# robertknight/ocrs-models

Measured on AMD Instinct MI355X. Metric: detection train-step images/sec, higher is better.
Workload: dtype bf16

## Files before the change

### ocrs_models_amd/csrc/det_mm.hip

```cpp
#include "det_common.h"
#include "det_rs.h"
#include <type_traits>

constexpr int mf_th(int cin, int cout, int nst) { return (nst != 2 && cin == 8 && cout != 32) ? 16 : 8; }

namespace {

template <int C>
struct MmPitch {
    static constexpr int V = (C == 32) ? 40 : C;
};

template <int CIN, int COUT, bool PPOOL = false>
struct MmCfg {
    static constexpr bool N256 = CIN == 32 && (COUT == 32 || COUT == 16);
    static constexpr int NT = N256 ? 256 : 512, NW = NT / 64;
    static constexpr int BPC = 2;
    static constexpr int TW = 32;
    static constexpr int TH = (CIN == 32 || COUT == 32) ? 8 : ((CIN == 16 && COUT == 16 && !PPOOL) ? 8 : 12);
    static constexpr bool MERGE = N256;
    static constexpr int TP = TW * TH;
    static constexpr bool T12P = CIN == 16 && COUT == 16 && TH == 12;
    static constexpr bool BDB = !(CIN == 8 && COUT == 16 && TH == 12) && !T12P && !N256;
    static constexpr int DW_ = TW + 2, DH_ = TH + 2, DP = DW_ * DH_;
    static constexpr int CGI = CIN / 8, CGO = COUT / 8;
    static constexpr int PD = MmPitch<COUT>::V, PX = MmPitch<CIN>::V;
    static constexpr int MT = (CIN + 15) / 16, NTO = (COUT + 15) / 16;
    static constexpr int KC = (9 * COUT + 31) / 32;
    static constexpr int NPW = TP / 16 / NW;
    static constexpr int KS = TP / 32;
    static constexpr int TAPU = (COUT == 8) ? 5 : 9;
    static constexpr int NOWN = (TAPU == 9) ? 8 / NW : 1;
    static constexpr int NGI = (DP * CGO + NT - 1) / NT;
    static constexpr int NXI = (TP * CGI + NT - 1) / NT;
    static constexpr int NWIN = (DH_ / 2) * (DW_ / 2);
    static constexpr int NWI = (NWIN * 2 * CGO + NT - 1) / NT;
    static_assert(DH_ % 2 == 0 && NT % (2 * CGO) == 0 && 4 * NWI <= 16, "pooled item layout");
    static constexpr int OFF_D = 0;
    static constexpr int OFF_X = (OFF_D + DP * PD * 2 + 63) & ~63;
    static constexpr int OFF_WF = (OFF_X + TP * PX * 2 + 64 + 63) & ~63;
    static constexpr int OFF_PAR = OFF_WF + MT * KC * 64 * 16;
    static constexpr int PAR_FLOATS = 3 * CIN + 6 * COUT + 9 * CIN + COUT * CIN + NW * 2 * MT * 16;
    static constexpr int TILE_BYTES = OFF_PAR + PAR_FLOATS * 4;
    static constexpr int SLOT_FLOATS = (NW * NOWN * MT * NTO + NW) * 256 + NW * 2 * MT * 16;
    static constexpr int SMEM = TILE_BYTES > SLOT_FLOATS * 4 ? TILE_BYTES : SLOT_FLOATS * 4;
    static constexpr int PART = COUT * CIN + 9 * CIN + 2 * CIN;
};

__device__ __forceinline__ f32x4 mfma16(const uint4& a, const uint4& b, f32x4 c) {
    return __builtin_amdgcn_mfma_f32_16x16x32_bf16(__builtin_bit_cast(bf16x8, a), __builtin_bit_cast(bf16x8, b), c, 0, 0, 0);
}
__device__ __forceinline__ f32x4 mfma16(const bf16x8& a, const bf16x8& b, f32x4 c) { return __builtin_amdgcn_mfma_f32_16x16x32_bf16(a, b, c, 0, 0, 0); }

__device__ __forceinline__ void half4(const Raw8<bf16>& r, int hf, float (&v)[4]) {
    const unsigned a = hf ? r.a.z : r.a.x, b = hf ? r.a.w : r.a.y;
    v[0] = __uint_as_float(a << 16); v[1] = __uint_as_float(a & 0xffff0000u);
    v[2] = __uint_as_float(b << 16); v[3] = __uint_as_float(b & 0xffff0000u);
}
__device__ __forceinline__ void st4bf(bf16* p, const float (&v)[4]) {
    unsigned lo, hi;
    asm("v_cvt_pk_bf16_f32 %0, %1, %2" : "=v"(lo) : "v"(v[0]), "v"(v[1]));
    asm("v_cvt_pk_bf16_f32 %0, %1, %2" : "=v"(hi) : "v"(v[2]), "v"(v[3]));
    *reinterpret_cast<uint2*>(p) = make_uint2(lo, hi);
}

typedef unsigned u32x4 __attribute__((ext_vector_type(4)));
__device__ __forceinline__ u32x4 gload16_opaque(const void* p) {
    u32x4 r;
    asm volatile("global_load_dwordx4 %0, %1, off" : "=&v"(r) : "v"(p) : "memory");
    return r;
}
template <int N>
__device__ __forceinline__ void wait_vm_tied(u32x4& r) {
    static_assert(N >= 0 && N < 64, "vmcnt is a 6-bit field");
    asm volatile("s_waitcnt vmcnt(%1)" : "+v"(r) : "n"(N) : "memory");
}
template <int NL, int NS, int K = 0>
__device__ __forceinline__ void static_for_wait(u32x4* v) {
    if constexpr (K < NL) {
        wait_vm_tied<NS + NL - 1 - K>(v[K]);
        static_for_wait<NL, NS, K + 1>(v);
    }
}
__device__ __forceinline__ Raw8<bf16> raw8_of(const u32x4& v) {
    Raw8<bf16> r;
    r.a = make_uint4(v.x, v.y, v.z, v.w);
    return r;
}

template <int CINB, int COUT>
constexpr int mm_fwd_lb() { return (CINB == 16 && COUT == 8) ? 6 : 4; }
template <int CINB, int COUT>
constexpr bool mm_fwd_fink() { return !(CINB == 16 && COUT == 8); }
template <int CIN, int COUT, bool PPOOL>
constexpr int mm_bwd_lb() { return MmCfg<CIN, COUT, PPOOL>::BPC * MmCfg<CIN, COUT, PPOOL>::NW / 4; }
}

template <int CIN, int COUT, bool PPOOL, bool G2, bool STATS, bool FULL = false>
__global__ __launch_bounds__((MmCfg<CIN, COUT, PPOOL>::NT), (mm_bwd_lb<CIN, COUT, PPOOL>())) void k_mm_bwd(Src2<bf16> x, const float* __restrict__ tra, const float* __restrict__ trb,
                                                   const float* __restrict__ wdw ,
                                                   const float* __restrict__ wpw , int ldw,
                                                   const bf16* __restrict__ g1, const bf16* __restrict__ g2, const bf16* __restrict__ z,
                                                   const float* __restrict__ bn, const float* __restrict__ coef, bf16* __restrict__ gxa,
                                                   bf16* __restrict__ gxb, float* __restrict__ ws, Tiling2 tg, BnFin fin, BwdLast bl) {
    using C = MmCfg<CIN, COUT, PPOOL>;
    constexpr int NT = C::NT, TW = C::TW, TH = C::TH, TP = C::TP, DW_ = C::DW_, DP = C::DP, CGI = C::CGI, CGO = C::CGO, PD = C::PD, PX = C::PX;
    constexpr int MT = C::MT, NTO = C::NTO, KC = C::KC, NPW = C::NPW, KS = C::KS;
    static_assert(!(FULL && PPOOL), "pooled launches have border tiles by construction (origin shift)");
    extern __shared__ __attribute__((aligned(64))) char smem[];
    bf16* tileD = reinterpret_cast<bf16*>(smem + C::OFF_D);
    bf16* tileX = reinterpret_cast<bf16*>(smem + C::OFF_X);
    uint4* s_wf = reinterpret_cast<uint4*>(smem + C::OFF_WF);
    float* s_trx = reinterpret_cast<float*>(smem + C::OFF_PAR);
    float* s_bn = s_trx + 3 * CIN;
    float* s_cf = s_bn + 3 * COUT;
    float* s_w9 = s_cf + 3 * COUT;
    float* s_wp = s_w9 + 9 * CIN;
    const int H = tg.H, W = tg.W;
    const int tid = threadIdx.x, lane = tid & 63, l15 = lane & 15;
    const int wave = __builtin_amdgcn_readfirstlane(tid >> 6);

    fill_tr8(s_trx, x, tra, trb, CIN, tid);
    for (int i = tid; i < 3 * COUT; i += NT) s_bn[i] = bn[i];
    if (fin.gsum) {
        bn_fin_coef(fin, COUT, s_cf, tid, NT, blockIdx.x == 0);
    } else {
        for (int i = tid; i < 3 * COUT; i += NT) s_cf[i] = coef[i];
    }
    for (int i = tid; i < 9 * CIN; i += NT) s_w9[i] = wdw[i];
    for (int i = tid; i < COUT * CIN; i += NT) s_wp[i] = wpw[(i / CIN) * ldw + (i % CIN)];
    {
        const uint4 z4 = make_uint4(0, 0, 0, 0);
        for (int i = tid; i < C::OFF_WF / 16; i += NT) reinterpret_cast<uint4*>(smem)[i] = z4;
    }
    __syncthreads();
    for (int f = tid; f < MT * KC * 64; f += NT) {
        const int l = f & 63, kc = (f >> 6) % KC, mt = (f >> 6) / KC;
        const int m = (FULL && CIN == 8) ? (l & 7) : mt * 16 + (l & 15);
        float v[8];
#pragma unroll
        for (int j = 0; j < 8; ++j) {
            const int k = kc * 32 + (l >> 4) * 8 + j, tap = k / COUT, o = k % COUT;
            v[j] = (m < CIN && tap < 9) ? s_w9[m * 9 + tap] * s_wp[o * CIN + m] : 0.f;
        }
        s_wf[f] = make_uint4(pack2bf(v[0], v[1]), pack2bf(v[2], v[3]), pack2bf(v[4], v[5]), pack2bf(v[6], v[7]));
    }
    __syncthreads();

    const int cgo = tid % CGO;
    constexpr int NQ = 2 * CGO;
    const int cq4 = (tid % NQ) * 4;
    int gi_dyx[PPOOL ? C::NWI : C::NGI];
    if constexpr (!PPOOL) {
#pragma unroll
        for (int j = 0; j < C::NGI; ++j) {
            const int d = (tid + j * NT) / CGO, dy = d / DW_, dx = d - dy * DW_;
            gi_dyx[j] = dy | (dx << 16);
        }
    } else {
#pragma unroll
        for (int j = 0; j < C::NWI; ++j) {
            const int wd = (tid + j * NT) / NQ, wy = wd / (DW_ / 2), wx = wd - wy * (DW_ / 2);
            gi_dyx[j] = (2 * wy) | ((2 * wx) << 16);
        }
    }
    const int cgi = tid % CGI;
    const bool xi_a = cgi * 8 < x.Ca;
    const bf16* xi_base = xi_a ? x.a + cgi * 8 : x.b + (cgi * 8 - x.Ca);
    const int xi_pitch = xi_a ? x.Ca : x.Cb;
    constexpr int ORG = PPOOL ? -1 : 0;

    constexpr int NG = PPOOL ? 1 : C::NGI, NP = PPOOL ? C::NWI : 1;
    constexpr int GW = G2 ? 3 : 2, NLOADS = NG * GW + C::NXI;
    constexpr int PFD = 1;
    u32x4 pf[PFD][NLOADS];
    constexpr int NSTORE = NPW * MT;
    uint2 zp[4 * NP], gp1[NP], gp2[G2 ? NP : 1];
    unsigned okg_[PFD], okx_[PFD];
#pragma unroll
    for (int q = 0; q < PFD; ++q) okg_[q] = okx_[q] = 0;
    auto ld16 = [&](const bf16* p) -> u32x4 {
        if constexpr (FULL) {
            return gload16_opaque(p);
        } else {
            const uint4 q = *reinterpret_cast<const uint4*>(p);
            return (u32x4){q.x, q.y, q.z, q.w};
        }
    };
    auto issue = [&](const TileOrg& o, auto SET) {
        constexpr int SI = decltype(SET)::value;
        unsigned okg = 0, okx = 0;
        const int h00 = o.h0 + ORG - 1, w00 = o.w0 + ORG - 1;
        const int corner = (o.n * H + h00) * W + w00;
        const bf16* zb = z + (long)corner * COUT;
        const bool inside = FULL && h00 >= 0 && w00 >= 0 && h00 + C::DH_ <= H && w00 + DW_ <= W;
        if constexpr (!PPOOL) {
            const bf16* g1b = g1 + (long)corner * COUT;
            const bf16* g2b = (G2 ? g2 : g1) + (long)corner * COUT;
            auto items = [&](auto INSIDE) {
#pragma unroll
// ... 47 lines not shown
        else xitems(std::false_type{});
        okg_[SI] = okg;
        okx_[SI] = okx;
    };

    const int kg = lane >> 4;
    auto tap_off = [](int tap) constexpr -> int { return tap < 9 ? ((2 - tap / 3) * DW_ + (2 - tap % 3)) * PD : 0; };
    auto boff_of = [&](int kc, bool& valid) -> int {
        if constexpr (COUT == 32) {
            valid = true;
            return tap_off(kc) + kg * 8;
        } else if constexpr (COUT == 16) {
            const int t0 = 2 * kc, t1 = 2 * kc + 1;
            valid = (kg < 2) ? t0 < 9 : t1 < 9;
            return ((kg < 2) ? tap_off(t0) : tap_off(t1)) + (kg & 1) * 8;
        } else {
            const int t0 = 4 * kc;
            valid = t0 + kg < 9;
            const int a = (kg & 1) ? tap_off(t0 + 1) : tap_off(t0), b = (kg & 1) ? tap_off(t0 + 3) : tap_off(t0 + 2);
            return (kg & 2) ? b : a;
        }
    };
    const int prow = 4 * (lane >> 4) + ((lane & 15) >> 2), pcol = (lane & 3) * 4;
    auto unit_off = [&](int u) -> int {
        if constexpr (COUT == 8) {
            const int sel = (lane & 3) >> 1;
            int tap = 2 * u + sel;
            tap = tap > 8 ? 8 : tap;
            const int ky = tap / 3, kx = tap - ky * 3;
            return ((2 - ky) * DW_ + prow + 2 - kx) * PD + (lane & 1) * 4;
        } else {
            const int ky = u / 3, kx = u - ky * 3;
            return ((2 - ky) * DW_ + prow + 2 - kx) * PD + pcol;
        }
    };
    constexpr int NSUB = MT * NTO, NKR = C::NW / NSUB;
    static_assert(C::NW % NSUB == 0 && KS >= NKR, "shared-unit split");
    const int u_own = (C::TAPU == 9) ? wave : (wave & 3);
    const int ks_own0 = (C::TAPU == 9) ? 0 : (wave >> 2) * (KS / 2), ks_own1 = (C::TAPU == 9) ? KS : ks_own0 + KS / 2;
    const int sh_a = (wave % NSUB) % MT, sh_b = (wave % NSUB) / MT, sh_k0 = (wave / NSUB) * KS / NKR, sh_k1 = (wave / NSUB + 1) * KS / NKR;
    constexpr int NOWN = C::NOWN;
    int off_own[NOWN];
#pragma unroll
    for (int j = 0; j < NOWN; ++j) off_own[j] = unit_off(u_own + j * C::NW);
    const int off_sh = unit_off(C::TAPU - 1) + sh_b * 16;
    f32x4 accO[NOWN][MT][NTO], accS = (f32x4){0.f, 0.f, 0.f, 0.f};
#pragma unroll
    for (int j = 0; j < NOWN; ++j)
#pragma unroll
        for (int a = 0; a < MT; ++a)
#pragma unroll
            for (int b = 0; b < NTO; ++b) accO[j][a][b] = (f32x4){0.f, 0.f, 0.f, 0.f};
    constexpr bool STL = STATS && (MT == 2 || C::T12P);
    float* s_st = s_wp + COUT * CIN;
    float st1[(STATS && !STL) ? MT : 1][4];
    if constexpr (STATS && !STL) {
#pragma unroll
        for (int a = 0; a < MT; ++a)
#pragma unroll
            for (int i = 0; i < 4; ++i) st1[a][i] = 0.f;
    }
    if constexpr (STL) {
        for (int i = tid; i < C::NW * 2 * MT * 16; i += NT) s_st[i] = 0.f;
    }

    TileSched ts(tg.ntiles);
    TileIter<TW, TH> tit(tg, ts.first < ts.end ? ts.first : 0, ts.step);
    TileOrg orgs[PFD];
    orgs[0] = tit.org();
    using I0 = std::integral_constant<int, 0>;
    if (ts.first < ts.end) issue(orgs[0], I0{});
    auto tile_body = [&](long t, auto KIND, auto SET) __attribute__((always_inline)) {
        constexpr int SI = decltype(SET)::value, KI = decltype(KIND)::value;
        const TileOrg org = orgs[SI];
        const unsigned okg = okg_[SI], okx = okx_[SI];
        if constexpr (FULL) {
            constexpr int YOUNGER = KI == 0 ? 0 : NSTORE;
            static_for_wait<NLOADS, YOUNGER>(pf[SI]);
        }
        if constexpr (!PPOOL) {
#pragma unroll
            for (int hf = 0; hf < 2; ++hf) {
                const int c4 = cgo * 8 + hf * 4;
                const f32x4 bs = *reinterpret_cast<const f32x4*>(s_bn + c4), bt = *reinterpret_cast<const f32x4*>(s_bn + COUT + c4);
                const f32x4 ca = *reinterpret_cast<const f32x4*>(s_cf + c4), cb = *reinterpret_cast<const f32x4*>(s_cf + COUT + c4),
                            cc = *reinterpret_cast<const f32x4*>(s_cf + 2 * COUT + c4);
#pragma unroll
                for (int j = 0; j < C::NGI; ++j) {
                    const int it = tid + j * NT;
                    if (DP * CGO % NT == 0 || it < DP * CGO) {
                        float dz[4] = {0.f, 0.f, 0.f, 0.f};
                        if (okg & (1u << j)) {
                            float zv[4], ga[4];
                            half4(raw8_of(pf[SI][j * GW + 0]), hf, zv);
                            half4(raw8_of(pf[SI][j * GW + 1]), hf, ga);
                            if constexpr (G2) {
                                float gb[4];
                                half4(raw8_of(pf[SI][j * GW + 2]), hf, gb);
#pragma unroll
                                for (int i = 0; i < 4; ++i) ga[i] += gb[i];
                            }
#pragma unroll
                            for (int i = 0; i < 4; ++i) {
                                const float gh = fmaf(zv[i], bs[i], bt[i]) > 0.f ? ga[i] : 0.f;
                                dz[i] = fmaf(ca[i], gh, fmaf(cb[i], zv[i], cc[i]));
                            }
                        }
// ... 340 lines not shown
    red[chain][col] = s;
    __syncthreads();
    __shared__ float fin[32];
    const float v = ((red[0][col] + red[1][col]) + (red[2][col] + red[3][col])) + ((red[4][col] + red[5][col]) + (red[6][col] + red[7][col]));
    if (chain == 0) fin[col] = v;
    __syncthreads();
    if (chain != 0 || e >= nelem) return;
    if (e >= COUT * CIN + 9 * CIN) {
        const int r2 = e - (COUT * CIN + 9 * CIN);
        if (r2 & 1) return;
        const int c = r2 >> 1, Cb = CIN - Ca;
        const bool in_a = c < Ca;
        double* gs = in_a ? gsum_a : gsum_b;
        if (!gs) return;
        const int cc = in_a ? c : c - Ca, Cs = in_a ? Ca : Cb;
        const float* sv = in_a ? saved_a : saved_b;
        const float* tr = in_a ? tra : trb;
        const double S1 = v, S2 = fin[col + 1], sc = tr[cc], sh = tr[Cs + cc], mean = sv[cc], rstd = sv[Cs + cc];
        gs[cc] += S1;
        if (sc != 0.0) gs[Cs + cc] += rstd * ((S2 - sh * S1) / sc - mean * S1);
        return;
    }
    if (e < COUT * CIN) {
        const int o = e / CIN, c = e - o * CIN;
        dwpw[o * ldw + c] += v;
        return;
    }
    const int r = e - COUT * CIN;
    if (r < 9 * CIN) {
        dwdw[r] += v;
        return;
    }
    return;
}
static int mm_grid(int th, int N, int H, int W, int pooled, int bpc = 2) {
    const long ntiles = (long)N * ((W + pooled + 31) / 32) * ((H + pooled + th - 1) / th);
    return persistent_grid(ntiles, bpc);
}
static int mm_bwd_th(int Cin, int Cout, int pooled) {
    if (Cin == 32 || Cout == 32) return 8;
    return (Cin == 16 && Cout == 16 && !pooled) ? 8 : 12;
}

template <int CIN, int COUT, bool PPOOL, bool G2, bool STATS>
static void mm_bwd_launch1(const Src2<bf16>& x, const float* tra, const float* trb, const float* wdw, const float* wpw, int ldw, const bf16* g1, const bf16* g2,
                           const bf16* z, const float* bn, const float* coef, bf16* gxa, bf16* gxb, float* ws, int N, int H, int W, int nb, const BnFin& fin,
                           const BwdLast& bl, hipStream_t st) {
    using CC = MmCfg<CIN, COUT, PPOOL>;
    Tiling2 tg = make_tiling2(N, H + (PPOOL ? 1 : 0), W + (PPOOL ? 1 : 0), CC::TW, CC::TH);
    tg.H = H;
    tg.W = W;
    if constexpr (!PPOOL) {
        if (W % CC::TW == 0) {
            hipFuncSetAttribute(reinterpret_cast<const void*>(&k_mm_bwd<CIN, COUT, PPOOL, G2, STATS, true>), hipFuncAttributeMaxDynamicSharedMemorySize, CC::SMEM);
            OCRS_LAUNCH_T((k_mm_bwd<CIN, COUT, PPOOL, G2, STATS, true>), dim3(nb), dim3(CC::NT), CC::SMEM, st, x, tra, trb, wdw, wpw, ldw, g1, g2, z, bn, coef,
                          gxa, gxb, ws, tg, fin, bl);
            return;
        }
    }
    hipFuncSetAttribute(reinterpret_cast<const void*>(&k_mm_bwd<CIN, COUT, PPOOL, G2, STATS, false>), hipFuncAttributeMaxDynamicSharedMemorySize, CC::SMEM);
    OCRS_LAUNCH_T((k_mm_bwd<CIN, COUT, PPOOL, G2, STATS, false>), dim3(nb), dim3(CC::NT), CC::SMEM, st, x, tra, trb, wdw, wpw, ldw, g1, g2, z, bn, coef, gxa, gxb,
                  ws, tg, fin, bl);
}

template <int CIN, int COUT>
static void mm_bwd_dispatch(const Src2<bf16>& x, const float* tra, const float* trb, const float* wdw, const float* wpw, int ldw, const bf16* g1, const bf16* g2,
                            int pooled, const bf16* z, const float* bn, const float* coef, bf16* gxa, bf16* gxb, float* ws, bool stats, int N, int H, int W,
                            int nb, const BnFin& fin, const BwdLast& bl, hipStream_t st) {
#define MMB(PP, GG, SS) mm_bwd_launch1<CIN, COUT, PP, GG, SS>(x, tra, trb, wdw, wpw, ldw, g1, g2, z, bn, coef, gxa, gxb, ws, N, H, W, nb, fin, bl, st)
    if (pooled) {
        if (g2) { if (stats) MMB(true, true, true); else MMB(true, true, false); }
        else    { if (stats) MMB(true, false, true); else MMB(true, false, false); }
    } else {
        if (g2) { if (stats) MMB(false, true, true); else MMB(false, true, false); }
        else    { if (stats) MMB(false, false, true); else MMB(false, false, false); }
    }
#undef MMB
}

static BwdLast mm_bwd_last(bool want, int Cin, int Ca, double* gsA, double* gsB, const float* svA, const float* svB) {
    BwdLast bl{nullptr, nullptr, gsA, gsB, svA, svB, Ca, 0};
    if (!want) return bl;
    double* p = bwd_defer_scratch(BWD_LAST_SLOTS * 2 * Cin + 2);
    if (p) {
        bl.raw = p;
        bl.counter = reinterpret_cast<unsigned*>(p + BWD_LAST_SLOTS * 2 * Cin);
    }
    return bl;
}
static void mm_bwd_second_stage(const float* ws, int nb, int Cin, int Cout, int Ca, float* dwpw, int ldw, float* dwdw, double* gsA, double* gsB, const float* svA,
                                const float* svB, const float* tA, const float* tB, const BwdLast& bl, bool may_defer, hipStream_t st) {
    const int ne = Cout * Cin + 11 * Cin;
    if (bl.raw) {
        gsA = gsB = nullptr;
        if (may_defer && bwd_defer_reduce(ws, nb, ne, dwpw, Cout * Cin, Cin, ldw, dwdw, 9 * Cin)) return;
    } else if (may_defer && !gsA && !gsB && bwd_defer_reduce(ws, nb, ne, dwpw, Cout * Cin, Cin, ldw, dwdw, 9 * Cin)) {
        return;
    }
    OCRS_LAUNCH_T(k_mm_bwd_reduce, dim3((ne + 31) / 32), dim3(256), 0, st, ws, nb, Cin, Cout, Ca, dwpw, ldw, dwdw, gsA, gsB, svA, svB, tA, tB);
}

extern "C" {

long ocrs_mm_bwd_supported(int Ca, int Cb, int Cout, int dtype) {
    if (dtype != 1 || !(Cout == 8 || Cout == 16 || Cout == 32)) return 0;
    const int Cin = Ca + Cb;
    if (Ca == 32 && Cb == 32) return 1;
    if ((Cin == 8 && Cout == 32) || (Cin == 32 && Cout == 8)) return 0;
    return (Cin == 8 || Cin == 16 || Cin == 32) && Ca % 8 == 0 && Cb % 8 == 0;
}
long ocrs_mm_bwd_ws_floats(int Ca, int Cb, int Cout, int N, int H, int W) {
    const int Cin = (Ca == 32 && Cb == 32) ? 32 : Ca + Cb;
    const int nb0 = mm_grid(mm_bwd_th(Cin, Cout, 0), N, H, W, 0), nb1 = mm_grid(mm_bwd_th(Cin, Cout, 1), N, H, W, 1);
    const long tiled = (long)(nb0 > nb1 ? nb0 : nb1) * (Cout * Cin + 11 * Cin + 1024) * ((Ca == 32 && Cb == 32) ? 2 : 1);
// ... 68 lines not shown
                       const float* bn, const double* gsum, const float* gamma, const float* saved, float* dgamma, float* dbeta, void* gxa, float* dwpw,
                       float* dwdw, float* ws, const float* saved_a, double* gsum_a, int Cout, int N, int H, int W, int dtype, hipStream_t st) {
    OCRS_CHECK_ARG(xu && wexp && tra && wdw && wpw && g1 && z && bn && gsum && gamma && saved && dgamma && dbeta && gxa && dwpw && dwdw && ws);
    OCRS_CHECK_ARG(ocrs_mm_bwd_head_supported(8, 0, Cout, N, H, W, dtype) && (!gsum_a || saved_a));
    const BnFin fin{gsum, gamma, saved, dgamma, dbeta, (long)N * H * W};
    Src2<bf16> x{nullptr, nullptr, 8, 0};
    const int nb = rs_bwd_blocks(8, Cout, N, H, W, g2 != nullptr);
    const BwdLast bl = mm_bwd_last(gsum_a != nullptr, 8, 8, gsum_a, nullptr, saved_a, nullptr);
    rs_bwd_launch(x, tra, nullptr, wdw, wpw, 8, (const bf16*)g1, (const bf16*)g2, (const bf16*)z, bn, nullptr, (bf16*)gxa, nullptr, ws, gsum_a != nullptr, Cout, N, H, W,
                  fin, st, nullptr, nullptr, (const bf16*)xu, wexp, bl);
    mm_bwd_second_stage(ws, nb, 8, Cout, 8, dwpw, 8, dwdw, gsum_a, nullptr, saved_a, nullptr, tra, nullptr, bl, true, st);
    OCRS_LAUNCH_CHECK();
    return OCRS_OK;
}

int ocrs_mm_bwd_fin_xu_c1(const void* xu, const float* wexp, const float* tra, const float* wdw, const float* wpw, const void* g1, const void* g2, const void* z,
                          const float* bn, const double* gsum, const float* gamma, const float* saved, float* dgamma, float* dbeta, float* dwpw, float* dwdw,
                          float* ws, const float* saved_a, double* gsum_a, const float* img, double* c1acc, int Cout, int N, int H, int W, int dtype,
                          hipStream_t st) {
    OCRS_CHECK_ARG(xu && wexp && tra && wdw && wpw && g1 && z && bn && gsum && gamma && saved && dgamma && dbeta && dwpw && dwdw && ws && img && c1acc);
    OCRS_CHECK_ARG(Cout == 8 && ocrs_mm_bwd_head_supported(8, 0, Cout, N, H, W, dtype) && (!gsum_a || saved_a));
    const BnFin fin{gsum, gamma, saved, dgamma, dbeta, (long)N * H * W};
    Src2<bf16> x{nullptr, nullptr, 8, 0};
    const int nb = rs_bwd_blocks(8, Cout, N, H, W, g2 != nullptr);
    const BwdLast bl = mm_bwd_last(gsum_a != nullptr, 8, 8, gsum_a, nullptr, saved_a, nullptr);
    rs_bwd_launch(x, tra, nullptr, wdw, wpw, 8, (const bf16*)g1, (const bf16*)g2, (const bf16*)z, bn, nullptr, nullptr, nullptr, ws, gsum_a != nullptr, Cout, N, H, W,
                  fin, st, nullptr, nullptr, (const bf16*)xu, wexp, bl, img, c1acc);
    mm_bwd_second_stage(ws, nb, 8, Cout, 8, dwpw, 8, dwdw, gsum_a, nullptr, saved_a, nullptr, tra, nullptr, bl, true, st);
    OCRS_LAUNCH_CHECK();
    return OCRS_OK;
}

int ocrs_mm_bwd(const void* xa, const void* xb, int Ca, int Cb, const float* tra, const float* trb, const float* wdw, const float* wpw, const void* g1,
                const void* g2, int pooled, const void* z, const float* bn, const float* coef, void* gxa, void* gxb, float* dwpw, float* dwdw, float* ws,
                const float* saved_a, double* gsum_a, const float* saved_b, double* gsum_b, int Cout, int N, int H, int W, int dtype, hipStream_t st) {
    const BnFin fin{nullptr, nullptr, nullptr, nullptr, nullptr, 0};
    return mm_bwd_impl(xa, xb, Ca, Cb, tra, trb, wdw, wpw, g1, g2, pooled, z, bn, coef, fin, gxa, gxb, dwpw, dwdw, ws, saved_a, gsum_a, saved_b, gsum_b, Cout, N, H,
                       W, dtype, st);
}

int ocrs_mm_bwd_fin(const void* xa, const void* xb, int Ca, int Cb, const float* tra, const float* trb, const float* wdw, const float* wpw, const void* g1,
                    const void* g2, int pooled, const void* z, const float* bn, const double* gsum, const float* gamma, const float* saved, float* dgamma,
                    float* dbeta, void* gxa, void* gxb, float* dwpw, float* dwdw, float* ws, const float* saved_a, double* gsum_a, const float* saved_b,
                    double* gsum_b, int Cout, int N, int H, int W, int dtype, hipStream_t st) {
    OCRS_CHECK_ARG(gsum && gamma && saved && dgamma && dbeta);
    const BnFin fin{gsum, gamma, saved, dgamma, dbeta, (long)N * H * W};
    return mm_bwd_impl(xa, xb, Ca, Cb, tra, trb, wdw, wpw, g1, g2, pooled, z, bn, nullptr, fin, gxa, gxb, dwpw, dwdw, ws, saved_a, gsum_a, saved_b, gsum_b, Cout, N,
                       H, W, dtype, st);
}

}

namespace {
template <int CINB, int NST, int COUT>
struct MfCfg {
    static constexpr int NT = 512, NW = 8;
    static constexpr int TW = 32, TH = mf_th(CINB, COUT, NST), TP = TW * TH;
    static constexpr int DW_ = TW + 2, DH_ = TH + 2, DP = DW_ * DH_;
    static constexpr int CGB = CINB / 8;
    static constexpr int PX = MmPitch<CINB>::V;
    static constexpr int MT = (COUT + 15) / 16;
    static constexpr int KC = (9 * CINB + 31) / 32;
    static_assert(TH % 8 == 0, "forward tiles: TH (row pair, column half) units over 8 waves");
    static constexpr int UPW = TH / 8, NPW = 2 * UPW;
    static constexpr int NXI = (DP * CGB + NT - 1) / NT;
    static constexpr int OFF_X = 0;
    static constexpr int OFF_WF = (DP * PX * 2 + 63) & ~63;
    static constexpr int OFF_PAR = OFF_WF + NST * MT * KC * 64 * 16;
    static constexpr int PAR_FLOATS = 3 * CINB * NST + 9 * CINB * NST + COUT * CINB * NST + NW * MT * 16 * 2;
    static constexpr int SMEM = OFF_PAR + PAR_FLOATS * 4;
};
}

template <bool AGENT>
__device__ __forceinline__ double bn_parts_chain_sum(const float* __restrict__ parts, int nparts, int C, int e, int chain) {
    double s = 0.0;
    if (e < 2 * C) {
        double a[8] = {0, 0, 0, 0, 0, 0, 0, 0};
        auto ld = [&](long i) -> double {
            if constexpr (AGENT) return (double)__hip_atomic_load(parts + i, __ATOMIC_RELAXED, __HIP_MEMORY_SCOPE_AGENT);
            else return (double)parts[i];
        };
        int b = chain;
        for (; b + 56 < nparts; b += 64) {
#pragma unroll
            for (int u = 0; u < 8; ++u) a[u] += ld((long)(b + 8 * u) * 2 * C + e);
        }
        for (int u = 0; b < nparts; b += 8, ++u) a[u & 7] += ld((long)b * 2 * C + e);
        s = ((a[0] + a[1]) + (a[2] + a[3])) + ((a[4] + a[5]) + (a[6] + a[7]));
    }
    return s;
}

struct XuSrc {
    const bf16* u;
    const float* wexp;
};
template <int CINB, int NST, int COUT, bool POOL, bool FULL, bool XU = false>
__global__ __launch_bounds__(512, (mm_fwd_lb<CINB, COUT>())) void k_mm_fwd(Src2<bf16> x, const float* __restrict__ tra, const float* __restrict__ trb,
                                                   const float* __restrict__ wdw , const float* __restrict__ wpw ,
                                                   bf16* __restrict__ z, float* __restrict__ ws , Tiling2 tg,
                                                   const float* __restrict__ gamma, bf16* __restrict__ pooled, FwdFin fin, XuSrc xu) {
    static_assert(!XU || (CINB == 8 && NST == 1), "u plane: the 8-channel output of the first block");
    using C = MfCfg<CINB, NST, COUT>;
    constexpr int NT = C::NT, TW = C::TW, TH = C::TH, DW_ = C::DW_, DP = C::DP, CGB = C::CGB, PX = C::PX, MT = C::MT, KC = C::KC, NPW = C::NPW;
    constexpr int CIN = CINB * NST;
    extern __shared__ __attribute__((aligned(64))) char smem[];
    bf16* tileX = reinterpret_cast<bf16*>(smem + C::OFF_X);
    uint4* s_wf = reinterpret_cast<uint4*>(smem + C::OFF_WF);
    float* s_trx = reinterpret_cast<float*>(smem + C::OFF_PAR);
    float* s_w9 = s_trx + 3 * CIN;
    float* s_wp = s_w9 + 9 * CIN;
    float* s_stat = s_wp + COUT * CIN;
    const int H = tg.H, W = tg.W;
    const int tid = threadIdx.x, lane = tid & 63, l15 = lane & 15;
    const int wave = __builtin_amdgcn_readfirstlane(tid >> 6);

    fill_tr8(s_trx, x, tra, trb, CIN, tid);
    for (int i = tid; i < 9 * CIN; i += NT) s_w9[i] = wdw[i];
    for (int i = tid; i < COUT * CIN; i += NT) s_wp[i] = wpw[i];
    {
        const uint4 z4 = make_uint4(0, 0, 0, 0);
        for (int i = tid; i < C::OFF_WF / 16; i += NT) reinterpret_cast<uint4*>(smem)[i] = z4;
    }
    __syncthreads();
    for (int f = tid; f < NST * MT * KC * 64; f += NT) {
        const int l = f & 63, kc = (f >> 6) % KC, mt = ((f >> 6) / KC) % MT, st = (f >> 6) / (KC * MT);
        const int m = (FULL && COUT == 8) ? (l & 7) : mt * 16 + (l & 15);
        float v[8];
#pragma unroll
        for (int j = 0; j < 8; ++j) {
            const int k = kc * 32 + (l >> 4) * 8 + j, tap = k / CINB, c = st * CINB + k % CINB;
            v[j] = (m < COUT && tap < 9) ? s_w9[c * 9 + tap] * s_wp[m * CIN + c] : 0.f;
        }
        s_wf[f] = make_uint4(pack2bf(v[0], v[1]), pack2bf(v[2], v[3]), pack2bf(v[4], v[5]), pack2bf(v[6], v[7]));
    }
    __syncthreads();

    const int cgb = tid % CGB;
    int xi_dyx[C::NXI];
#pragma unroll
    for (int j = 0; j < C::NXI; ++j) {
        const int d = (tid + j * NT) / CGB, dy = d / DW_, dx = d - dy * DW_;
        xi_dyx[j] = dy | (dx << 16);
    }
    u32x4 xr[NST][C::NXI];
    float we[XU ? 8 : 1];
    if constexpr (XU) {
#pragma unroll
        for (int i = 0; i < 8; ++i) we[i] = xu.wexp[i];
    }
    unsigned okx = 0;
    constexpr int NSTORE = NPW * MT + (POOL ? (NPW / 2) * MT : 0);
    constexpr int NLOAD = NST * C::NXI;
    auto issue = [&](const TileOrg& o) {
        okx = 0;
        const int corner = (o.n * H + (o.h0 - 1)) * W + (o.w0 - 1);
#pragma unroll
        for (int st = 0; st < NST; ++st) {
            const int c0 = st * CINB + cgb * 8;
            const bool in_a = c0 < x.Ca;
            const bf16* base = in_a ? x.a + c0 : x.b + (c0 - x.Ca);
            const int pitch = in_a ? x.Ca : x.Cb;
            const bf16* cb = base + (long)corner * pitch;
            auto items = [&](auto INSIDE) {
#pragma unroll
                for (int j = 0; j < C::NXI; ++j) {
                    const int dy = xi_dyx[j] & 0xffff, dx = xi_dyx[j] >> 16, h = o.h0 - 1 + dy, w = o.w0 - 1 + dx;
                    const bool it_ok = (j + 1) * NT <= DP * CGB || tid + j * NT < DP * CGB;
                    const bool ok = it_ok && (decltype(INSIDE)::value || ((unsigned)h < (unsigned)H && (unsigned)w < (unsigned)W));
                    const bf16* src = XU ? (ok ? xu.u + ((corner + dy * W + dx) & ~7) : xu.u) : (ok ? cb + (dy * W + dx) * pitch : base);
                    if constexpr (FULL) {
                        xr[st][j] = gload16_opaque(src);
                    } else {
                        const uint4 q = *reinterpret_cast<const uint4*>(src);
                        xr[st][j] = (u32x4){q.x, q.y, q.z, q.w};
                    }
                    okx |= ok ? 1u << (st * C::NXI + j) : 0u;
                }
            };
            if (FULL && o.h0 >= 1 && o.w0 >= 1 && o.h0 + TH + 1 <= H && o.w0 + TW + 1 <= W) items(std::true_type{});
            else items(std::false_type{});
        }
    };
    auto wait_loads = [&](bool pend_stores) {
        if constexpr (FULL) {
            if (pend_stores) {
                static_for_wait<NLOAD, NSTORE>(&xr[0][0]);
            } else {
                static_for_wait<NLOAD, 0>(&xr[0][0]);
// ... 207 lines not shown
    if (!fin.counter) return;
    asm volatile("s_waitcnt vmcnt(0)" ::: "memory");
    __syncthreads();
    int* s_flag = reinterpret_cast<int*>(smem);
    double* red = reinterpret_cast<double*>(smem + 64);
    if (tid == 0) *s_flag = __hip_atomic_fetch_add(fin.counter, 1u, __ATOMIC_RELAXED, __HIP_MEMORY_SCOPE_AGENT) == gridDim.x - 1 ? 1 : 0;
    __syncthreads();
    if (*s_flag == 0) return;
    static_assert(2 * COUT <= 64 && NT == 512, "two 32-element windows x 8 chains x 32 columns = the 512 threads");
    const int win = tid >> 8, t8 = tid & 255, col = t8 & 31, chain = t8 >> 5, e = win * 32 + col;
    red[(win * 8 + chain) * 32 + col] = bn_parts_chain_sum<true>(ws, gridDim.x, COUT, e, chain);
    __syncthreads();
    if (chain == 0) {
        const double* r = red + win * 256;
        const double tot = ((r[col] + r[32 + col]) + (r[64 + col] + r[96 + col])) + ((r[128 + col] + r[160 + col]) + (r[192 + col] + r[224 + col]));
        red[512 + win * 32 + col] = tot;
    }
    __syncthreads();
    if (tid == 0) {
        if (fin.nbt) *fin.nbt += 1;
        __hip_atomic_store(fin.counter, 0u, __ATOMIC_RELAXED, __HIP_MEMORY_SCOPE_AGENT);
    }
    if (chain == 0 && e < 2 * COUT && !(e & 1))
        bn_finalize_channel(red[512 + e], red[512 + e + 1], fin.count, e >> 1, COUT, fin.gamma, fin.beta, fin.eps, fin.momentum, fin.tr, fin.saved, fin.run_mean,
                            fin.run_var, fin.lo);
}

__global__ __launch_bounds__(256) void k_bn_finalize_parts(const float* __restrict__ parts, int nparts, long count, int C, const float* __restrict__ gamma,
                                                           const float* __restrict__ beta, float eps, float momentum, float* __restrict__ tr,
                                                           float* __restrict__ saved, float* __restrict__ run_mean, float* __restrict__ run_var,
                                                           long long* __restrict__ nbt, float lo) {
    __shared__ double red[8][32];
    const int col = threadIdx.x & 31, chain = threadIdx.x >> 5;
    const int e = blockIdx.x * 32 + col;
    red[chain][col] = bn_parts_chain_sum<false>(parts, nparts, C, e, chain);
    __syncthreads();
    if (chain != 0) return;
    const double tot = ((red[0][col] + red[1][col]) + (red[2][col] + red[3][col])) + ((red[4][col] + red[5][col]) + (red[6][col] + red[7][col]));
    red[0][col] = tot;
    __syncthreads();
    if (e == 0 && nbt) *nbt += 1;
    if (e >= 2 * C || (e & 1)) return;
    bn_finalize_channel(tot, red[0][col + 1], count, e >> 1, C, gamma, beta, eps, momentum, tr, saved, run_mean, run_var, lo);
}

template <int CINB, int NST, int COUT>
static void mm_fwd_launch(const Src2<bf16>& x, const float* tra, const float* trb, const float* wdw, const float* wpw, bf16* z, float* ws, const float* gamma,
                          bf16* pooled, int N, int H, int W, int nb, const FwdFin& fin, hipStream_t st, const XuSrc& xu = XuSrc{nullptr, nullptr}) {
    using CC = MfCfg<CINB, NST, COUT>;
    const Tiling2 tg = make_tiling2(N, H, W, CC::TW, CC::TH);
    const bool full = H % CC::TH == 0 && W % CC::TW == 0 && (!pooled || ((H | W) & 1) == 0);
#define MF_LAUNCH(PO_, FU_)                                                                                                                          \
    {                                                                                                                                                \
        hipFuncSetAttribute(reinterpret_cast<const void*>(&k_mm_fwd<CINB, NST, COUT, PO_, FU_>), hipFuncAttributeMaxDynamicSharedMemorySize, CC::SMEM); \
        hipLaunchKernelGGL((k_mm_fwd<CINB, NST, COUT, PO_, FU_>), dim3(nb), dim3(CC::NT), CC::SMEM, st, x, tra, trb, wdw, wpw, z, ws, tg, gamma, pooled, fin, xu); \
    }
    if constexpr (CINB == 8 && NST == 1) {
        if (xu.u) {
#define MF_LAUNCH_XU(FU_)                                                                                                                                 \
    {                                                                                                                                                     \
        hipFuncSetAttribute(reinterpret_cast<const void*>(&k_mm_fwd<CINB, NST, COUT, false, FU_, true>), hipFuncAttributeMaxDynamicSharedMemorySize, CC::SMEM); \
        hipLaunchKernelGGL((k_mm_fwd<CINB, NST, COUT, false, FU_, true>), dim3(nb), dim3(CC::NT), CC::SMEM, st, x, tra, trb, wdw, wpw, z, ws, tg, gamma, pooled, fin, xu); \
    }
            if (full) MF_LAUNCH_XU(true) else MF_LAUNCH_XU(false)
#undef MF_LAUNCH_XU
            return;
        }
    }
    if (pooled) {
        if (full) MF_LAUNCH(true, true) else MF_LAUNCH(true, false)
    } else {
        if (full) MF_LAUNCH(false, true) else MF_LAUNCH(false, false)
    }
#undef MF_LAUNCH
}

extern "C" {

long ocrs_mm_fwd_supported(int Ca, int Cb, int Cout, int dtype) {
    if (dtype != 1 || !(Cout == 8 || Cout == 16 || Cout == 32)) return 0;
    const int Cin = Ca + Cb;
    if (Ca == 32 && Cb == 32) return Cout == 32;
    if ((Cin == 8 && Cout == 32) || (Cin == 32 && Cout == 8)) return 0;
    return (Cin == 8 || Cin == 16 || Cin == 32) && Ca % 8 == 0 && Cb % 8 == 0;
}
long ocrs_mm_fwd_nparts(int Ca, int Cb, int Cout, int N, int H, int W) {
    if (rs_fwd_supported(Ca, Cb, Cout, N, H, W)) return rs_fwd_blocks(N, H, W);
    const int cinb = (Ca == 32 && Cb == 32) ? 32 : Ca + Cb;
    const int th = mf_th(cinb, Cout, (Ca == 32 && Cb == 32) ? 2 : 1);
    return mm_grid(th, N, H, W, 0, (cinb == 16 && Cout == 8) ? 3 : 2);
}

static int mm_fwd_impl(const void* xa, const void* xb, int Ca, int Cb, const float* tra, const float* trb, const float* wdw, const float* wpw, void* z, float* ws,
                       const float* gamma, void* pooled, int Cout, int N, int H, int W, int dtype, const FwdFin& fin, hipStream_t st,
                       const XuSrc& xu = XuSrc{nullptr, nullptr}) {
    OCRS_CHECK_ARG((xa || xu.u) && tra && wdw && wpw && z && ws && (Cb == 0 || (xb && trb)) && (!pooled || gamma));
    OCRS_CHECK_ARG(ocrs_mm_fwd_supported(Ca, Cb, Cout, dtype) && (long)N * (H + 2) * (W + 2) < (1L << 31));
    const int Cin = Ca + Cb;
    Src2<bf16> x{(const bf16*)xa, (const bf16*)xb, Ca, Cb};
    const int nb = (int)ocrs_mm_fwd_nparts(Ca, Cb, Cout, N, H, W);
    if (!pooled && rs_fwd_supported(Ca, Cb, Cout, N, H, W)) {
        rs_fwd_launch(x, xu.u, xu.wexp, tra, trb, wdw, wpw, (bf16*)z, ws, Cout, N, H, W, nb, fin, st);
        OCRS_LAUNCH_CHECK();
        return OCRS_OK;
    }
#define MF_CASE(CB_, NS_, CO_) \
    if (Cin == CB_ * NS_ && Cout == CO_ && (NS_ == 1 || Ca == 32)) mm_fwd_launch<CB_, NS_, CO_>(x, tra, trb, wdw, wpw, (bf16*)z, ws, gamma, (bf16*)pooled, N, H, W, nb, fin, st, xu);
    MF_CASE(8, 1, 8) MF_CASE(8, 1, 16) MF_CASE(16, 1, 8) MF_CASE(16, 1, 16) MF_CASE(16, 1, 32) MF_CASE(32, 1, 16) MF_CASE(32, 1, 32) MF_CASE(32, 2, 32)
// ... 41 lines not shown
```

Measured before the change: 2709.

## Widen 32-channel LDS tile pitch to avoid bank conflicts, alias weight staging

Changes the LDS row pitch for 32-channel tiles from 40 to 48 bf16 elements. A compile-time bank model says this makes the fragment and transposed reads conflict-free. To absorb the extra LDS, the 32x32 backward and 32x2 forward kernels place the fused weight fragments at the start of LDS and stage the float weight tables inside the tile area. The tiles are zeroed only after the fragments are built, which costs one extra barrier. A few configurations keep the old 40 pitch, and static asserts check LDS occupancy limits.

```diff
diff --git a/ocrs_models_amd/csrc/det_mm.hip b/ocrs_models_amd/csrc/det_mm.hip
--- a/ocrs_models_amd/csrc/det_mm.hip
+++ b/ocrs_models_amd/csrc/det_mm.hip
@@ -1,17 +1,32 @@
 #include "det_common.h"
 #include "det_rs.h"
+#include "lds_banks.h"
 #include <type_traits>
 
 constexpr int mf_th(int cin, int cout, int nst) { return (nst != 2 && cin == 8 && cout != 32) ? 16 : 8; }
 
 namespace {
 
-template <int C>
+template <int C, int P32>
 struct MmPitch {
-    static constexpr int V = (C == 32) ? 40 : C;
+    static_assert(P32 == lds::mm_pitch(32) || P32 == 40, "64-byte rows: + 32 bytes, or the former + 16");
+    static constexpr int V = (C == 32) ? P32 : lds::mm_pitch(C);
+    static constexpr bool FREE = lds::frag_read_cycles(V * 2) == lds::FRAG_FREE && lds::tr_read_cycles(V * 2) == lds::TR_FREE;
+    static_assert(C < 16 || FREE == !(C == 32 && P32 == 40), "tile pitch: reads conflict-free (2-way only with the former pad)");
 };
-
-template <int CIN, int COUT, bool PPOOL = false>
+template <int CIN, int COUT, bool PPOOL, bool G2, bool STATS, bool FULL>
+constexpr int mm_bwd_p32() {
+    if (CIN == 32 && COUT == 32 && !PPOOL && G2) return 40;
+    if (CIN == 16 && COUT == 32 && !PPOOL && G2 && STATS && !FULL) return 40;
+    return lds::mm_pitch(32);
+}
+template <int CINB, int NST, int COUT, bool POOL, bool FULL>
+constexpr int mm_fwd_p32() {
+    if (CINB == 32 && NST == 2 && POOL && !FULL) return 40;
+    return lds::mm_pitch(32);
+}
+
+template <int CIN, int COUT, bool PPOOL = false, int P32 = lds::mm_pitch(32)>
 struct MmCfg {
     static constexpr bool N256 = CIN == 32 && (COUT == 32 || COUT == 16);
     static constexpr int NT = N256 ? 256 : 512, NW = NT / 64;
@@ -24,7 +39,7 @@
     static constexpr bool BDB = !(CIN == 8 && COUT == 16 && TH == 12) && !T12P && !N256;
     static constexpr int DW_ = TW + 2, DH_ = TH + 2, DP = DW_ * DH_;
     static constexpr int CGI = CIN / 8, CGO = COUT / 8;
-    static constexpr int PD = MmPitch<COUT>::V, PX = MmPitch<CIN>::V;
+    static constexpr int PD = MmPitch<COUT, P32>::V, PX = MmPitch<CIN, P32>::V;
     static constexpr int MT = (CIN + 15) / 16, NTO = (COUT + 15) / 16;
     static constexpr int KC = (9 * COUT + 31) / 32;
     static constexpr int NPW = TP / 16 / NW;
@@ -36,12 +51,19 @@
     static constexpr int NWIN = (DH_ / 2) * (DW_ / 2);
     static constexpr int NWI = (NWIN * 2 * CGO + NT - 1) / NT;
     static_assert(DH_ % 2 == 0 && NT % (2 * CGO) == 0 && 4 * NWI <= 16, "pooled item layout");
-    static constexpr int OFF_D = 0;
+    static constexpr bool WALIAS = CIN == 32 && COUT == 32 && P32 != 40;
+    static constexpr int WF_BYTES = MT * KC * 64 * 16;
+    static constexpr int OFF_D = WALIAS ? WF_BYTES : 0;
     static constexpr int OFF_X = (OFF_D + DP * PD * 2 + 63) & ~63;
-    static constexpr int OFF_WF = (OFF_X + TP * PX * 2 + 64 + 63) & ~63;
-    static constexpr int OFF_PAR = OFF_WF + MT * KC * 64 * 16;
-    static constexpr int PAR_FLOATS = 3 * CIN + 6 * COUT + 9 * CIN + COUT * CIN + NW * 2 * MT * 16;
+    static constexpr int TILES_END = (OFF_X + TP * PX * 2 + 64 + 63) & ~63;
+    static constexpr int OFF_WF = WALIAS ? 0 : TILES_END;
+    static constexpr int OFF_PAR = WALIAS ? TILES_END : OFF_WF + WF_BYTES;
+    static_assert(OFF_WF + WF_BYTES - 1024 < 65536, "fragment reads: 16-bit offset field");
+    static constexpr int W_FLOATS = 9 * CIN + COUT * CIN;
+    static constexpr int PAR_FLOATS = 3 * CIN + 6 * COUT + (WALIAS ? 0 : W_FLOATS) + NW * 2 * MT * 16;
+    static_assert(!WALIAS || W_FLOATS * 4 <= TILES_END - OFF_D, "the staged weight tables lie inside the tile area");
     static constexpr int TILE_BYTES = OFF_PAR + PAR_FLOATS * 4;
+    static_assert(BPC * TILE_BYTES <= 160 * 1024, "resident workgroups per CU: LDS");
     static constexpr int SLOT_FLOATS = (NW * NOWN * MT * NTO + NW) * 256 + NW * 2 * MT * 16;
     static constexpr int SMEM = TILE_BYTES > SLOT_FLOATS * 4 ? TILE_BYTES : SLOT_FLOATS * 4;
     static constexpr int PART = COUT * CIN + 9 * CIN + 2 * CIN;
@@ -103,7 +125,7 @@
                                                    const bf16* __restrict__ g1, const bf16* __restrict__ g2, const bf16* __restrict__ z,
                                                    const float* __restrict__ bn, const float* __restrict__ coef, bf16* __restrict__ gxa,
                                                    bf16* __restrict__ gxb, float* __restrict__ ws, Tiling2 tg, BnFin fin, BwdLast bl) {
-    using C = MmCfg<CIN, COUT, PPOOL>;
+    using C = MmCfg<CIN, COUT, PPOOL, mm_bwd_p32<CIN, COUT, PPOOL, G2, STATS, FULL>()>;
     constexpr int NT = C::NT, TW = C::TW, TH = C::TH, TP = C::TP, DW_ = C::DW_, DP = C::DP, CGI = C::CGI, CGO = C::CGO, PD = C::PD, PX = C::PX;
     constexpr int MT = C::MT, NTO = C::NTO, KC = C::KC, NPW = C::NPW, KS = C::KS;
     static_assert(!(FULL && PPOOL), "pooled launches have border tiles by construction (origin shift)");
@@ -114,7 +136,7 @@
     float* s_trx = reinterpret_cast<float*>(smem + C::OFF_PAR);
     float* s_bn = s_trx + 3 * CIN;
     float* s_cf = s_bn + 3 * COUT;
-    float* s_w9 = s_cf + 3 * COUT;
+    float* s_w9 = C::WALIAS ? reinterpret_cast<float*>(smem + C::OFF_D) : s_cf + 3 * COUT;
     float* s_wp = s_w9 + 9 * CIN;
     const int H = tg.H, W = tg.W;
     const int tid = threadIdx.x, lane = tid & 63, l15 = lane & 15;
@@ -129,10 +151,11 @@
     }
     for (int i = tid; i < 9 * CIN; i += NT) s_w9[i] = wdw[i];
     for (int i = tid; i < COUT * CIN; i += NT) s_wp[i] = wpw[(i / CIN) * ldw + (i % CIN)];
-    {
+    auto zero_tiles = [&]() {
         const uint4 z4 = make_uint4(0, 0, 0, 0);
-        for (int i = tid; i < C::OFF_WF / 16; i += NT) reinterpret_cast<uint4*>(smem)[i] = z4;
-    }
+        for (int i = tid; i < (C::TILES_END - C::OFF_D) / 16; i += NT) reinterpret_cast<uint4*>(smem + C::OFF_D)[i] = z4;
+    };
+    if constexpr (!C::WALIAS) zero_tiles();
     __syncthreads();
     for (int f = tid; f < MT * KC * 64; f += NT) {
         const int l = f & 63, kc = (f >> 6) % KC, mt = (f >> 6) / KC;
@@ -146,6 +169,10 @@
         s_wf[f] = make_uint4(pack2bf(v[0], v[1]), pack2bf(v[2], v[3]), pack2bf(v[4], v[5]), pack2bf(v[6], v[7]));
     }
     __syncthreads();
+    if constexpr (C::WALIAS) {
+        zero_tiles();
+        __syncthreads();
+    }
 
     const int cgo = tid % CGO;
     constexpr int NQ = 2 * CGO;
@@ -299,7 +326,7 @@
 #pragma unroll
             for (int b = 0; b < NTO; ++b) accO[j][a][b] = (f32x4){0.f, 0.f, 0.f, 0.f};
     constexpr bool STL = STATS && (MT == 2 || C::T12P);
-    float* s_st = s_wp + COUT * CIN;
+    float* s_st = s_cf + 3 * COUT + (C::WALIAS ? 0 : C::W_FLOATS);
     float st1[(STATS && !STL) ? MT : 1][4];
     if constexpr (STATS && !STL) {
 #pragma unroll
@@ -746,14 +773,16 @@
     tg.W = W;
     if constexpr (!PPOOL) {
         if (W % CC::TW == 0) {
-            hipFuncSetAttribute(reinterpret_cast<const void*>(&k_mm_bwd<CIN, COUT, PPOOL, G2, STATS, true>), hipFuncAttributeMaxDynamicSharedMemorySize, CC::SMEM);
-            OCRS_LAUNCH_T((k_mm_bwd<CIN, COUT, PPOOL, G2, STATS, true>), dim3(nb), dim3(CC::NT), CC::SMEM, st, x, tra, trb, wdw, wpw, ldw, g1, g2, z, bn, coef,
+            constexpr int SMEM = MmCfg<CIN, COUT, PPOOL, mm_bwd_p32<CIN, COUT, PPOOL, G2, STATS, true>()>::SMEM;
+            hipFuncSetAttribute(reinterpret_cast<const void*>(&k_mm_bwd<CIN, COUT, PPOOL, G2, STATS, true>), hipFuncAttributeMaxDynamicSharedMemorySize, SMEM);
+            OCRS_LAUNCH_T((k_mm_bwd<CIN, COUT, PPOOL, G2, STATS, true>), dim3(nb), dim3(CC::NT), SMEM, st, x, tra, trb, wdw, wpw, ldw, g1, g2, z, bn, coef,
                           gxa, gxb, ws, tg, fin, bl);
             return;
         }
     }
-    hipFuncSetAttribute(reinterpret_cast<const void*>(&k_mm_bwd<CIN, COUT, PPOOL, G2, STATS, false>), hipFuncAttributeMaxDynamicSharedMemorySize, CC::SMEM);
-    OCRS_LAUNCH_T((k_mm_bwd<CIN, COUT, PPOOL, G2, STATS, false>), dim3(nb), dim3(CC::NT), CC::SMEM, st, x, tra, trb, wdw, wpw, ldw, g1, g2, z, bn, coef, gxa, gxb,
+    constexpr int SMEM = MmCfg<CIN, COUT, PPOOL, mm_bwd_p32<CIN, COUT, PPOOL, G2, STATS, false>()>::SMEM;
+    hipFuncSetAttribute(reinterpret_cast<const void*>(&k_mm_bwd<CIN, COUT, PPOOL, G2, STATS, false>), hipFuncAttributeMaxDynamicSharedMemorySize, SMEM);
+    OCRS_LAUNCH_T((k_mm_bwd<CIN, COUT, PPOOL, G2, STATS, false>), dim3(nb), dim3(CC::NT), SMEM, st, x, tra, trb, wdw, wpw, ldw, g1, g2, z, bn, coef, gxa, gxb,
                   ws, tg, fin, bl);
 }
 
@@ -928,23 +957,29 @@
 }
 
 namespace {
-template <int CINB, int NST, int COUT>
+template <int CINB, int NST, int COUT, int P32 = lds::mm_pitch(32)>
 struct MfCfg {
     static constexpr int NT = 512, NW = 8;
     static constexpr int TW = 32, TH = mf_th(CINB, COUT, NST), TP = TW * TH;
     static constexpr int DW_ = TW + 2, DH_ = TH + 2, DP = DW_ * DH_;
     static constexpr int CGB = CINB / 8;
-    static constexpr int PX = MmPitch<CINB>::V;
+    static constexpr int PX = MmPitch<CINB, P32>::V;
     static constexpr int MT = (COUT + 15) / 16;
     static constexpr int KC = (9 * CINB + 31) / 32;
     static_assert(TH % 8 == 0, "forward tiles: TH (row pair, column half) units over 8 waves");
     static constexpr int UPW = TH / 8, NPW = 2 * UPW;
     static constexpr int NXI = (DP * CGB + NT - 1) / NT;
-    static constexpr int OFF_X = 0;
-    static constexpr int OFF_WF = (DP * PX * 2 + 63) & ~63;
-    static constexpr int OFF_PAR = OFF_WF + NST * MT * KC * 64 * 16;
-    static constexpr int PAR_FLOATS = 3 * CINB * NST + 9 * CINB * NST + COUT * CINB * NST + NW * MT * 16 * 2;
+    static constexpr bool WALIAS = CINB == 32 && NST == 2 && P32 != 40;
+    static constexpr int WF_BYTES = NST * MT * KC * 64 * 16, X_BYTES = (DP * PX * 2 + 63) & ~63;
+    static constexpr int OFF_X = WALIAS ? WF_BYTES : 0;
+    static constexpr int OFF_WF = WALIAS ? 0 : X_BYTES;
+    static constexpr int OFF_PAR = X_BYTES + WF_BYTES;
+    static_assert(OFF_WF + WF_BYTES - 1024 < 65536, "fragment reads: 16-bit offset field");
+    static constexpr int W_FLOATS = 9 * CINB * NST + COUT * CINB * NST;
+    static constexpr int PAR_FLOATS = 3 * CINB * NST + (WALIAS ? 0 : W_FLOATS) + NW * MT * 16 * 2;
+    static_assert(!WALIAS || W_FLOATS * 4 <= X_BYTES, "the staged weight tables lie inside the tile area");
     static constexpr int SMEM = OFF_PAR + PAR_FLOATS * 4;
+    static_assert((mm_fwd_lb<CINB, COUT>() / 2) * SMEM <= 160 * 1024, "resident workgroups per CU: LDS");
 };
 }
 
@@ -978,16 +1013,16 @@
                                                    bf16* __restrict__ z, float* __restrict__ ws , Tiling2 tg,
                                                    const float* __restrict__ gamma, bf16* __restrict__ pooled, FwdFin fin, XuSrc xu) {
     static_assert(!XU || (CINB == 8 && NST == 1), "u plane: the 8-channel output of the first block");
-    using C = MfCfg<CINB, NST, COUT>;
+    using C = MfCfg<CINB, NST, COUT, mm_fwd_p32<CINB, NST, COUT, POOL, FULL>()>;
     constexpr int NT = C::NT, TW = C::TW, TH = C::TH, DW_ = C::DW_, DP = C::DP, CGB = C::CGB, PX = C::PX, MT = C::MT, KC = C::KC, NPW = C::NPW;
     constexpr int CIN = CINB * NST;
     extern __shared__ __attribute__((aligned(64))) char smem[];
     bf16* tileX = reinterpret_cast<bf16*>(smem + C::OFF_X);
     uint4* s_wf = reinterpret_cast<uint4*>(smem + C::OFF_WF);
     float* s_trx = reinterpret_cast<float*>(smem + C::OFF_PAR);
-    float* s_w9 = s_trx + 3 * CIN;
+    float* s_w9 = C::WALIAS ? reinterpret_cast<float*>(smem + C::OFF_X) : s_trx + 3 * CIN;
     float* s_wp = s_w9 + 9 * CIN;
-    float* s_stat = s_wp + COUT * CIN;
+    float* s_stat = s_trx + 3 * CIN + (C::WALIAS ? 0 : C::W_FLOATS);
     const int H = tg.H, W = tg.W;
     const int tid = threadIdx.x, lane = tid & 63, l15 = lane & 15;
     const int wave = __builtin_amdgcn_readfirstlane(tid >> 6);
@@ -995,10 +1030,11 @@
     fill_tr8(s_trx, x, tra, trb, CIN, tid);
     for (int i = tid; i < 9 * CIN; i += NT) s_w9[i] = wdw[i];
     for (int i = tid; i < COUT * CIN; i += NT) s_wp[i] = wpw[i];
-    {
+    auto zero_tile = [&]() {
         const uint4 z4 = make_uint4(0, 0, 0, 0);
-        for (int i = tid; i < C::OFF_WF / 16; i += NT) reinterpret_cast<uint4*>(smem)[i] = z4;
-    }
+        for (int i = tid; i < C::X_BYTES / 16; i += NT) reinterpret_cast<uint4*>(smem + C::OFF_X)[i] = z4;
+    };
+    if constexpr (!C::WALIAS) zero_tile();
     __syncthreads();
     for (int f = tid; f < NST * MT * KC * 64; f += NT) {
         const int l = f & 63, kc = (f >> 6) % KC, mt = ((f >> 6) / KC) % MT, st = (f >> 6) / (KC * MT);
@@ -1012,6 +1048,10 @@
         s_wf[f] = make_uint4(pack2bf(v[0], v[1]), pack2bf(v[2], v[3]), pack2bf(v[4], v[5]), pack2bf(v[6], v[7]));
     }
     __syncthreads();
+    if constexpr (C::WALIAS) {
+        zero_tile();
+        __syncthreads();
+    }
 
     const int cgb = tid % CGB;
     int xi_dyx[C::NXI];
@@ -1325,8 +1365,9 @@
     const bool full = H % CC::TH == 0 && W % CC::TW == 0 && (!pooled || ((H | W) & 1) == 0);
 #define MF_LAUNCH(PO_, FU_)                                                                                                                          \
     {                                                                                                                                                \
-        hipFuncSetAttribute(reinterpret_cast<const void*>(&k_mm_fwd<CINB, NST, COUT, PO_, FU_>), hipFuncAttributeMaxDynamicSharedMemorySize, CC::SMEM); \
-        hipLaunchKernelGGL((k_mm_fwd<CINB, NST, COUT, PO_, FU_>), dim3(nb), dim3(CC::NT), CC::SMEM, st, x, tra, trb, wdw, wpw, z, ws, tg, gamma, pooled, fin, xu); \
+        constexpr int SMEM = MfCfg<CINB, NST, COUT, mm_fwd_p32<CINB, NST, COUT, PO_, FU_>()>::SMEM;                                                  \
+        hipFuncSetAttribute(reinterpret_cast<const void*>(&k_mm_fwd<CINB, NST, COUT, PO_, FU_>), hipFuncAttributeMaxDynamicSharedMemorySize, SMEM);  \
+        hipLaunchKernelGGL((k_mm_fwd<CINB, NST, COUT, PO_, FU_>), dim3(nb), dim3(CC::NT), SMEM, st, x, tra, trb, wdw, wpw, z, ws, tg, gamma, pooled, fin, xu); \
     }
     if constexpr (CINB == 8 && NST == 1) {
         if (xu.u) {
diff --git a/ocrs_models_amd/csrc/lds_banks.h b/ocrs_models_amd/csrc/lds_banks.h
--- /dev/null
+++ b/ocrs_models_amd/csrc/lds_banks.h
@@ -0,0 +1,91 @@
+#pragma once
+
+namespace lds {
+
+enum Op { READ_B128, READ_B64, READ_B64_TR_B16, WRITE_B64, WRITE_B128 };
+
+struct OpDesc {
+    int ngroups;
+    int banks;
+    int bytes;
+    unsigned long long group[8];
+};
+
+constexpr OpDesc op_desc(Op op) {
+    switch (op) {
+        case READ_B128: {
+            const unsigned long long g0 = 0x0FF0F00FULL, g1 = 0xF00F0FF0ULL;
+            return OpDesc{4, 64, 16, {g0, g1, g0 << 32, g1 << 32, 0, 0, 0, 0}};
+        }
+        case READ_B64:
+        case READ_B64_TR_B16:
+            return OpDesc{2, 64, 8, {0xFFFFFFFFULL, 0xFFFFFFFFULL << 32, 0, 0, 0, 0, 0, 0}};
+        case WRITE_B64:
+            return OpDesc{4, 32, 8, {0xFFFFULL, 0xFFFFULL << 16, 0xFFFFULL << 32, 0xFFFFULL << 48, 0, 0, 0, 0}};
+        case WRITE_B128:
+        default:
+            return OpDesc{8, 32, 16, {0xFFULL, 0xFFULL << 8, 0xFFULL << 16, 0xFFULL << 24, 0xFFULL << 32, 0xFFULL << 40, 0xFFULL << 48, 0xFFULL << 56}};
+    }
+}
+
+template <class Map>
+constexpr int wave_cycles(Op op, Map map) {
+    const OpDesc d = op_desc(op);
+    int total = 0;
+    for (int g = 0; g < d.ngroups; ++g) {
+        int dw[128] = {};
+        int n = 0;
+        for (int lane = 0; lane < 64; ++lane) {
+            if (!((d.group[g] >> lane) & 1ULL)) continue;
+            const int a = map(lane);
+            for (int k = 0; k < d.bytes / 4; ++k) {
+                const int w = a / 4 + k;
+                bool seen = false;
+                for (int i = 0; i < n; ++i) seen = seen || dw[i] == w;
+                if (!seen) dw[n++] = w;
+            }
+        }
+        int worst = 0;
+        for (int i = 0; i < n; ++i) {
+            int cnt = 0;
+            for (int j = 0; j < n; ++j) cnt += (dw[j] % d.banks == dw[i] % d.banks) ? 1 : 0;
+            worst = cnt > worst ? cnt : worst;
+        }
+        total += worst;
+    }
+    return total;
+}
+
+struct FragMap {
+    int pitch;
+    constexpr int operator()(int lane) const { return (lane & 15) * pitch + (lane >> 4) * 16; }
+};
+struct TrMap {
+    int pitch;
+    constexpr int operator()(int lane) const { return (4 * (lane >> 4) + ((lane & 15) >> 2)) * pitch + (lane & 3) * 8; }
+};
+struct CommitMap {
+    int pitch, row, bytes;
+    constexpr int operator()(int lane) const { return (lane * bytes / row) * pitch + (lane * bytes) % row; }
+};
+constexpr int frag_read_cycles(int pitch) { return wave_cycles(READ_B128, FragMap{pitch}); }
+constexpr int tr_read_cycles(int pitch) { return wave_cycles(READ_B64_TR_B16, TrMap{pitch}); }
+constexpr int FRAG_FREE = 4, TR_FREE = 2;
+
+constexpr int mm_pitch(int C) { return C == 32 ? 48 : C; }
+constexpr bool pitch_free(int pitch_elems, bool transposed) {
+    return frag_read_cycles(pitch_elems * 2) == FRAG_FREE && (!transposed || tr_read_cycles(pitch_elems * 2) == TR_FREE);
+}
+static_assert(pitch_free(mm_pitch(16), true) && pitch_free(mm_pitch(32), true), "det_mm tile pitches");
+struct TilePitch {
+    const char* tile;
+    int channels, pitch_bytes;
+    bool transposed;
+};
+constexpr TilePitch TILE_PITCHES[] = {
+    {"det_mm x / dz tile", 16, mm_pitch(16) * 2, true},
+    {"det_mm x / dz tile", 32, mm_pitch(32) * 2, true},
+};
+static_assert(frag_read_cycles(80) == 8 && tr_read_cycles(80) == 4, "the row + 16-byte pad is 2-way conflicted on gfx950");
+
+}
```

Result: no change. 2731 (median of 6 runs) (+0.8%).
